# JGCRI/xanthos

Measured on AMD Instinct MI355X. Metric: cell-months/sec (pm_abcd_mrtm, 67,420 cells), higher is better.
Workload: dtype f64

## Files before the change

include/xanthos_hip.h:

```cpp
#ifndef XANTHOS_HIP_H
#define XANTHOS_HIP_H

#include <stddef.h>
#include <stdint.h>

#ifdef __cplusplus
extern "C" {
#endif

#define XH_OK 0
#define XH_ERR_ARG 1
#define XH_ERR_HIP 2
#define XH_ERR_LIMIT 3
#define XH_ERR_DEVICE 4

#define XH_MAX_LCS 32

typedef struct xh_ctx xh_ctx;
typedef struct xh_route_plan xh_route_plan;

int xh_abi_version(void);
int xh_device_count(int *n);
int xh_ctx_create(int device, xh_ctx **out);
void xh_ctx_destroy(xh_ctx *ctx);
// ... 83 lines not shown

int xh_gwam(xh_ctx *ctx, int64_t ncell, int32_t nmonths, int32_t spinup, int32_t precip_col_spinup,
            int32_t precip_col_sim, double indexing,
            const double *d_pet, const double *d_precip,
            const double *d_sm_max, const double *d_sm0,
            double *d_aet, double *d_q, double *d_sav,
            double *d_sm_end);

int xh_route_plan_create(xh_ctx *ctx, int64_t ncell, const int64_t *h_indptr, const int32_t *h_indices,
                         const int8_t *h_sign, xh_route_plan **out);
void xh_route_plan_destroy(xh_route_plan *plan);
int xh_route_plan_info(const xh_route_plan *plan, int64_t info[16]);

int xh_route_plan_prepare(xh_ctx *ctx, xh_route_plan *plan, const double *h_flow_dist, const double *h_velocity, double dt);

int xh_route_plan_stats(xh_route_plan *plan, int64_t max_words, uint64_t *h_words, int64_t *n_words);

int xh_mrtm_downstream(int64_t ncell, int32_t nrow, int32_t ncol, const int64_t *h_id, const int32_t *h_ilon,
                       const int32_t *h_ilat, const double *h_flowdir, int64_t *h_dsid);
int xh_mrtm_upstream(int64_t ncell, int32_t nrow, int32_t ncol, const int64_t *h_id, const int32_t *h_ilon,
                     const int32_t *h_ilat, const int64_t *h_dsid, int64_t *h_upid);
int xh_mrtm_um_csr(int64_t ncell, const int64_t *h_upid, int64_t *h_indptr, int32_t *h_indices, int8_t *h_sign);

#define XH_ROUTE_DEFAULT 0
#define XH_ROUTE_FORCE_FALLBACK 1
#define XH_ROUTE_ATOMIC 2
#define XH_ROUTE_NO_DATAFLOW 4
#define XH_ROUTE_NO_SKEW 8
#define XH_ROUTE_TEST_FAULT 16
#define XH_ROUTE_VALIDATE 32
#define XH_ROUTE_REASSOC 128
#define XH_ROUTE_EXACT 256
int xh_route_plan_rsum_info(const xh_route_plan *plan, int64_t info[8]);
int xh_route_series(xh_ctx *ctx, xh_route_plan *plan, int32_t nmonths, int32_t spinup_months,
                    const int32_t *h_ndays, double dt,
                    const double *d_flow_dist, const double *d_velocity, const double *d_area,
                    const double *d_runoff, const double *d_S0,
                    double *d_chstorage, double *d_avgchflow, double *d_S_end, double *d_F_end, int32_t flags);

typedef struct xh_fused_args {
    int64_t ncell;
    int32_t nmonths, start_year;
    const xh_pm_tables *pm;
    int32_t n_lc_years;
    const int32_t *h_lc_years;
    int32_t water_idx, snow_idx;
    const double *d_tas, *d_tmin, *d_rhs, *d_wind, *d_rsds, *d_rlds, *d_tairprev, *d_lct, *d_elev;
    int32_t abcd_spinup, n_groups;
    const int32_t *h_basin_index, *h_par_index;
    int64_t npar_rows;
    const double *d_pars, *d_precip, *d_abcd_tmin;
    xh_route_plan *plan;
    int32_t routing_spinup;
    const int32_t *h_ndays;
    double dt;
    const double *d_flow_dist, *d_velocity, *d_area, *d_S0;
    int32_t route_flags;
    double *d_pet, *d_aet, *d_q, *d_sav, *d_chstorage, *d_avgchflow;
    int32_t block_months;
    int32_t mode;
} xh_fused_args;
int xh_run_fused(xh_ctx *ctx, const xh_fused_args *args);

int xh_calib_objective(xh_ctx *ctx, int64_t ncell_b, int32_t nmonths, int32_t spinup, int32_t nmembers,
                       int32_t npar, const double *h_pars, const double *d_pet_t, const double *d_precip_t,
                       const double *d_tmin_t, const double *d_area, const double *h_obs, double *h_ed,
// ... 163 lines not shown
```

xanthos_amd/_hip.py:

```python
import contextlib
import ctypes
import os
import threading
from ctypes import POINTER, Structure, byref, c_char_p, c_double, c_int, c_int8, c_int32, c_int64, c_size_t, \
    c_uint64, c_void_p

import numpy as np

_HERE = os.path.dirname(os.path.abspath(__file__))
LIB_PATH = os.environ.get('XH_LIBRARY') or os.path.join(_HERE, 'libxanthos_hip.so')

XH_ROUTE_DEFAULT, XH_ROUTE_FORCE_FALLBACK, XH_ROUTE_ATOMIC, XH_ROUTE_NO_DATAFLOW, XH_ROUTE_NO_SKEW = 0, 1, 2, 4, 8
XH_ROUTE_TEST_FAULT, XH_ROUTE_VALIDATE = 16, 32
XH_ROUTE_REASSOC, XH_ROUTE_EXACT = 128, 256
XH_ROUTE_NO_PLAIN = 0x4000
XH_DAYLIGHT_REFERENCE, XH_DAYLIGHT_MONTHLY = 0, 1
XH_ERR_ARG, XH_ERR_HIP, XH_ERR_LIMIT, XH_ERR_DEVICE = 1, 2, 3, 4
ENS_STAT_BITS = {'mean': 1, 'std': 2, 'min': 4, 'max': 8}


class HipUnavailable(RuntimeError):
    """The HIP library or device is not usable; nothing falls back to the CPU."""


# ... 70 lines not shown
    'xh_memcpy_d2d': (c_int, [_P, _P, _P, c_size_t]),
    'xh_host_alloc': (c_int, [_P, c_size_t, POINTER(c_void_p)]),
    'xh_host_free': (c_int, [_P, _P]),
    'xh_memcpy_h2d_async': (c_int, [_P, _P, _P, c_size_t]),
    'xh_memcpy_d2h_async': (c_int, [_P, _P, _P, c_size_t]),
    'xh_upload_file': (c_int, [_P, _P, c_char_p, ctypes.c_uint64, c_size_t, c_int]),
    'xh_download_file': (c_int, [_P, _P, c_char_p, ctypes.c_uint64, c_size_t, c_int]),
    'xh_download_files': (c_int, [_P, c_int, POINTER(c_void_p), POINTER(c_char_p), POINTER(ctypes.c_uint64), POINTER(c_size_t)]),
    'xh_csv_format': (c_int, [_P, _P, c_int64, c_int64, c_int64, _P, c_size_t, _P]),
    'xh_csv_write': (c_int, [_P, _P, c_int64, c_int64, c_int64, c_char_p, ctypes.c_uint64, c_size_t, POINTER(ctypes.c_uint64)]),
    'xh_csv_write_many': (c_int, [_P, c_int, POINTER(c_void_p), POINTER(c_int64), POINTER(c_int64), POINTER(c_int64),
                                  POINTER(c_char_p), POINTER(ctypes.c_uint64), c_size_t, POINTER(ctypes.c_uint64)]),
    'xh_pack_f32_be': (c_int, [_P, _P, c_int64, _P]),
    'xh_memset': (c_int, [_P, _P, c_int, c_size_t]),
    'xh_sync': (c_int, [_P]),
    'xh_gather_rows': (c_int, [_P, _P, _P, c_int64, c_int64, _P]),
    'xh_scatter_rows': (c_int, [_P, _P, _P, c_int64, c_int64, _P]),
    'xh_transpose': (c_int, [_P, _P, c_int64, c_int64, _P]),
    'xh_timing_reset': (c_int, [_P]),
    'xh_timing_enable': (c_int, [_P, c_int]),
    'xh_timing_get': (c_int, [_P, c_char_p, POINTER(c_double), POINTER(c_int64)]),
    'xh_pm_pet': (c_int, [_P, POINTER(PmTables), c_int64, c_int32, c_int32, c_int32, _P, c_int32, c_int32,
                          _P, _P, _P, _P, _P, _P, _P, _P, _P, _P]),
    'xh_abcd': (c_int, [_P, c_int64, c_int32, c_int32, c_int32, _P, _P, c_int64, _P, _P, _P, _P, _P, _P, _P, _P, _P]),
    'xh_hargreaves_pet': (c_int, [_P, c_int64, c_int32, _P, _P, _P, _P, _P, _P, _P]),
    'xh_gwam': (c_int, [_P, c_int64, c_int32, c_int32, c_int32, c_int32, c_double, _P, _P, _P, _P, _P, _P, _P, _P]),
    'xh_hs_pet': (c_int, [_P, c_int64, c_int32, _P, _P, _P, _P, _P, _P]),
    'xh_thornthwaite_pet': (c_int, [_P, c_int64, c_int32, c_int32, c_int32, _P, _P, _P, _P]),
    'xh_route_plan_create': (c_int, [_P, c_int64, _P, _P, _P, POINTER(c_void_p)]),
    'xh_route_plan_destroy': (None, [_P]),
    'xh_route_plan_info': (c_int, [_P, POINTER(c_int64)]),
    'xh_route_plan_stats': (c_int, [_P, c_int64, _P, POINTER(c_int64)]),
    'xh_route_plan_rsum_info': (c_int, [_P, POINTER(c_int64)]),
    'xh_route_plan_prepare': (c_int, [_P, _P, _P, _P, c_double]),
    'xh_mrtm_downstream': (c_int, [c_int64, c_int32, c_int32, _P, _P, _P, _P, _P]),
    'xh_mrtm_upstream': (c_int, [c_int64, c_int32, c_int32, _P, _P, _P, _P, _P]),
    'xh_mrtm_um_csr': (c_int, [c_int64, _P, _P, _P, _P]),
    'xh_route_series': (c_int, [_P, _P, c_int32, c_int32, _P, c_double, _P, _P, _P, _P, _P, _P, _P, _P, _P, c_int32]),
    'xh_run_fused': (c_int, [_P, POINTER(FusedArgs)]),
    'xh_calib_objective': (c_int, [_P, c_int64, c_int32, c_int32, c_int32, c_int32, _P, _P, _P, _P, _P, _P, _P, _P]),
    'xh_calib_objective_multi': (c_int, [_P, c_int32, _P, c_int32, c_int32, c_int32, c_int32, _P, _P, _P, _P, _P, _P, _P, _P]),
    'xh_calib_de_create': (c_int, [_P, c_int32, _P, _P, c_int32, c_int32, c_int32, c_int32, _P, _P, _P, _P, _P, _P, _P,
                                   c_uint64, POINTER(c_void_p)]),
    'xh_calib_flow_objective_multi': (c_int, [_P, c_int32, _P, c_int32, c_int32, c_int32, c_int32, _P, _P, _P, _P,
                                              POINTER(CalibFlowDesc), _P, _P, _P]),
    'xh_calib_de_create_flow': (c_int, [_P, c_int32, _P, _P, c_int32, c_int32, c_int32, c_int32, _P, _P, _P,
                                        POINTER(CalibFlowDesc), _P, _P, _P, c_uint64, POINTER(c_void_p)]),
    'xh_calib_gauge_objective_multi': (c_int, [_P, c_int32, _P, c_int32, c_int32, c_int32, c_int32, _P, _P, _P, _P,
                                               POINTER(CalibGaugeDesc), _P, _P, _P, _P]),
    'xh_calib_de_create_gauge': (c_int, [_P, c_int32, _P, _P, c_int32, c_int32, c_int32, c_int32, _P, _P, _P,
                                         POINTER(CalibGaugeDesc), _P, _P, _P, c_uint64, POINTER(c_void_p)]),
    'xh_calib_flow_velocity_objective_multi': (c_int, [_P, c_int32, _P, c_int32, c_int32, c_int32, c_int32, _P, _P, _P, _P,
                                                       POINTER(CalibFlowDesc), POINTER(CalibVelocityDesc), _P, _P, _P]),
    'xh_calib_gauge_velocity_objective_multi': (c_int, [_P, c_int32, _P, c_int32, c_int32, c_int32, c_int32, _P, _P, _P, _P,
                                                        POINTER(CalibGaugeDesc), POINTER(CalibVelocityDesc), _P, _P, _P,
                                                        _P]),
    'xh_calib_de_create_flow_velocity': (c_int, [_P, c_int32, _P, _P, c_int32, c_int32, c_int32, c_int32, _P, _P, _P,
                                                 POINTER(CalibFlowDesc), POINTER(CalibVelocityDesc), _P, _P, _P, c_uint64,
                                                 POINTER(c_void_p)]),
    'xh_calib_de_create_gauge_velocity': (c_int, [_P, c_int32, _P, _P, c_int32, c_int32, c_int32, c_int32, _P, _P, _P,
                                                  POINTER(CalibGaugeDesc), POINTER(CalibVelocityDesc), _P, _P, _P, c_uint64,
                                                  POINTER(c_void_p)]),
    'xh_calib_de_destroy': (None, [_P]),
    'xh_calib_de_init': (c_int, [_P]),
    'xh_calib_de_step': (c_int, [_P, c_int32, c_double, c_double, c_double, c_double, c_double, POINTER(c_int32)]),
    'xh_calib_de_result': (c_int, [_P, _P, _P, _P, _P, _P]),
# ... 586 lines not shown


class RoutePlan:

    def __init__(self, ctx, indptr, indices, sign):
        self.ctx = ctx
        ip = np.ascontiguousarray(indptr, dtype=np.int64)
        ix = np.ascontiguousarray(indices, dtype=np.int32)
        sg = np.ascontiguousarray(sign, dtype=np.int8)
        self.ncell = ip.size - 1
        h = c_void_p()
        ctx._check(lib().xh_route_plan_create(ctx.handle, self.ncell, _host_ptr(ip), _host_ptr(ix), _host_ptr(sg),
                                              byref(h)))
        self.handle = h.value

    def info(self):
        arr = (c_int64 * 16)()
        self.ctx._check(lib().xh_route_plan_info(self.handle, arr))
        keys = ('networks', 'largest_network', 'units', 'fallback_cells', 'largest_unit', 'slots', 'single_downstream',
                'flow_units', 'flow_edges', 'flow_depth', 'flow_cells', 'flow_max_imports', 'skew_max_lag',
                'last_tree_kernel', 'reroutes', 'validated')
        return dict(zip(keys, list(arr)))

    def prepare(self, flow_dist, velocity, dt):
        L = np.ascontiguousarray(flow_dist, dtype=np.float64)
        v = np.ascontiguousarray(velocity, dtype=np.float64)
        if L.size != self.ncell or v.size != self.ncell:
            raise ValueError('flow_dist / velocity must have one value per cell')
        self.ctx._check(lib().xh_route_plan_prepare(self.ctx.handle, self.handle, _host_ptr(L), _host_ptr(v), float(dt)))

    def rsum_info(self):
        arr = (c_int64 * 8)()
        self.ctx._check(lib().xh_route_plan_rsum_info(self.handle, arr))
        return dict(zip(('units', 'folded', 'fold_disabled', 'prepared_folded', 'pair_cells', 'prepared_pair_cells', 'guard_trips',
                         'pair_units'), list(arr)))

    def stats(self):
        n = c_int64(0)
        self.ctx._check(lib().xh_route_plan_stats(self.handle, 0, None, byref(n)))
        if n.value == 0:
            return None
        out = np.empty(n.value, dtype=np.uint64)
        self.ctx._check(lib().xh_route_plan_stats(self.handle, n.value, _host_ptr(out), byref(n)))
        return out.reshape(-1, 6)

    def close(self):
        if self.handle is not None and self.ctx.handle is not None:
            lib().xh_route_plan_destroy(self.handle)
        self.handle = None

    def __del__(self):
        try:
            self.close()
        except Exception:
            pass


def comm_unique_id():
    buf = ctypes.create_string_buffer(128)
    _check_host(lib().xh_comm_unique_id(buf, 128))
    return buf.raw


class Comm:

    def __init__(self, ctx, nranks, rank, unique_id):
        self.ctx, self.nranks, self.rank = ctx, int(nranks), int(rank)
        h = c_void_p()
# ... 200 lines not shown
```

xanthos_amd/csrc/xh_flow_rsum.cpp:

```cpp
#include <algorithm>
#include <cstdio>
#include <numeric>
#include <string>
#include <thread>

#include "xh_flow_plan.h"

using xh_flow::Tree;
using xh_flow::tree_analyse;

namespace {

constexpr int LANES = 64;
constexpr int G_MAX = 16;
constexpr int W_MAX = 9;
constexpr int SK_P = 4;
constexpr unsigned SK_ZERO = 2u * LANES * 16u;
constexpr int H_MAX = 88;

struct RPart {
    std::vector<int> queue, piece, roots, psize, pimp, pdepth;
    std::vector<int> e_prod, e_cons, e_kind;
    std::vector<int> unit_of_piece, unit_cells, unit_imp, unit_out, unit_depth;
    std::vector<char> unit_cheap, unit_special, special, mayfire;
// ... 560 lines not shown
            hs[out.unit_p[u] & 3]++;
            hl[std::min(out.unit_lmax[u] / 16, 13)]++;
            hi[P.unit_imp[u] == 0 ? 0 : P.unit_imp[u] <= 2 ? 1 : P.unit_imp[u] <= 4 ? 2 : P.unit_imp[u] <= 8 ? 3 : 4]++;
            indep += (P.unit_imp[u] == 0 && unit_exp[u] == 0) ? 1 : 0;
        }
        fprintf(stderr, "flow plan (reassociated): %d units (%d without streams, %d kept cheap), %d pieces, %d streams, depth %d, %lld of %lld lanes used\n",
                nunit, indep, P.n_cheap, (int)roots.size(), nedge, P.maxdepth + 1, (long long)out.n_cells, (long long)ts);
        {
            int nfu = 0, nfi = 0;
            for (int u = 0; u < nunit; ++u) {
                nfu += (out.unit_p[u] & 4) ? 1 : 0;
                nfi += ((out.unit_p[u] & 4) && (P.unit_imp[u] > 0 || unit_exp[u] > 0)) ? 1 : 0;
            }
            fprintf(stderr, "  folded leaves: %d, in %d units (of them with streams: %d)\n", out.n_folded, nfu, nfi);
        }
        {
            int nsu = 0;
            for (int u = 0; u < nunit; ++u) nsu += (out.unit_p[u] & 16) ? 1 : 0;
            int nx = 0;
            for (int c = 0; c < n; ++c) nx += (P.n_special >= 0 && P.mayfire[c]) ? 1 : 0;
            int quiet = 0;
            for (int u = 0; u < nunit && P.n_special >= 0; ++u) {
                bool any = (out.unit_p[u] & 16) != 0;
                for (int k = 0; k < LANES && !any; ++k) any = (out.lane_flags[(int64_t)u * LANES + k] & 1) != 0;
                quiet += any ? 0 : 1;
            }
            for (int u = 0; u < nunit && P.n_special >= 0; ++u)
                if (out.unit_p[u] & 16)
                    fprintf(stderr, "  pair unit %d: %d cells, %d imports, %d outlets, depth %d, lmax %d\n", u, P.unit_cells[u], P.unit_imp[u], unit_exp[u],
                            P.unit_depth[u], out.unit_lmax[u]);
            fprintf(stderr, "  single-sum plan: %s, %d cells may fire, %d of them in pair form in %d units; %d single units hold no cell that may fire\n",
                    P.n_special >= 0 ? "yes" : "no", nx, std::max(P.n_special, 0), nsu, quiet);
        }
        fprintf(stderr, "  units by reads (none, A, R, A+R): %d %d %d %d\n  units by lmax/16 (0..13+):", hs[0], hs[1], hs[2], hs[3]);
        for (int k = 0; k < 14; ++k) fprintf(stderr, " %d", hl[k]);
        fprintf(stderr, "\n  units by imports (0, <=2, <=4, <=8, more): %d %d %d %d %d\n  longest stream jump: %d levels\n", hi[0], hi[1],
                hi[2], hi[3], hi[4], out.skew_span);
    }
    return 0;
}

std::string flow_tables_check_rsum(int n, const int64_t *indptr, const int32_t *indices, const int8_t *sign,
                                   const std::vector<char> &handled, const FlowTables &t) {
    if (!t.rsum) return "not a reassociated plan";
    if (t.n_units == 0) {
        for (int c = 0; c < n; ++c)
            if (handled[c]) return "handled cell without units";
        return "";
    }
    const int64_t ts = (int64_t)t.n_units * LANES;
    if ((int64_t)t.cell_of_slot.size() != ts || (int64_t)t.lag.size() != ts || (int64_t)t.eprev.size() != ts ||
        (int64_t)t.ent2.size() != 2 * SK_P * ts || (int)t.unit_p.size() != t.n_units || (int64_t)t.ghost_edge.size() != ts ||
        (int64_t)t.ghost_lag.size() != ts || (int64_t)t.export_edge.size() != ts || (int)t.unit_lmax.size() != t.n_units ||
        (int)t.unit_order.size() != t.n_units || (int)t.edge_cons_unit.size() != t.n_edges ||
        (int)t.edge_prod_cell.size() != t.n_edges || (int)t.edge_cons_cell.size() != t.n_edges || (int)t.ds.size() != n ||
        (int)t.unit_depth.size() != t.n_units)
        return "table sizes";
    std::vector<int> slot_of(n, -1);
    for (int64_t s = 0; s < ts; ++s) {
        const int c = t.cell_of_slot[s];
        if (c < 0) continue;
        if (c >= n || !handled[c]) return "slot holds a cell that is not handled";
        if (slot_of[c] >= 0) return "cell " + std::to_string(c) + " sits in two slots";
        slot_of[c] = (int)s;
    }
    std::vector<int> carrier(n, -1);
// ... 148 lines not shown
```

xanthos_amd/csrc/xh_mrtm.hip:

```cpp
#include <algorithm>
#include <chrono>
#include <climits>
#include <cmath>
#include <atomic>
#include <numeric>
#include <thread>

#include "xh_common.h"
#include <sys/stat.h>
#include <unistd.h>

#include "xh_mrtm_flow.h"
#include "xh_mrtm_plan.h"

namespace {

constexpr int W_MAX = 9;
constexpr int W_BASE = 3;
constexpr int UNIT_MAX_CELLS = 3072;
constexpr int BIN_CELLS = 256;
constexpr int N_CLASS = XH_ROUTE_N_CLASS;

struct UnitClass {
    int nt, kc;
// ... 747 lines not shown
            prepared.first_checked = false;
        }
        plan->fold_tried = true;
        plan->prep_key = key;
        plan->fold_disabled = false;
        const bool fold = fold_on && nfold > 0;
        if (!fold && !single_on) return XH_OK;
        const int rcu = rsum_partition(ctx, plan, fold ? foldable.data() : nullptr, single_on ? capable.data() : nullptr,
                                       &prepared.fp);
        if (rcu || !prepared.fp) return rcu;
        prepared.suffix = prepared.fp->n_special >= 0 ? "_rs" : "_rf";
        plan->fold_dt = dt;
        return XH_OK;
    }
    return XH_OK;
}

void xh_route_backoff(xh_route_plan *plan) {
    plan->fault_streak = std::min(plan->fault_streak + 1, 6);
    plan->skip_calls = 4 << plan->fault_streak;
}

extern "C" int xh_route_plan_rsum_info(const xh_route_plan *plan, int64_t info[8]) {
    if (!plan || !info) return XH_ERR_ARG;
    const FlowPlan *fp = last_reassoc(plan), *prep = plan->form[XH_FORM_PREPARED].fp;
    info[0] = fp ? fp->n_units : 0;
    info[1] = fp ? fp->n_folded : 0;
    info[2] = plan->fold_disabled ? 1 : 0;
    info[3] = prep ? prep->n_folded : 0;
    info[4] = fp ? fp->n_special : -1;
    info[5] = prep ? prep->n_special : -1;
    info[6] = plan->guard_trips;
    info[7] = fp ? fp->n_pair_units : 0;
    return XH_OK;
}

RouteChoice route_choose(const xh_route_plan *plan, int flags, double dt, bool fed) {
    RouteChoice c;
    c.whole_graph = (flags & XH_ROUTE_FORCE_FALLBACK) != 0;
    c.atomic = (flags & XH_ROUTE_ATOMIC) != 0;
    c.dataflow = !c.whole_graph && plan->form[XH_FORM_EXACT].fp && (flags & XH_ROUTE_NO_DATAFLOW) == 0;
    c.skew = (flags & XH_ROUTE_NO_SKEW) == 0;
    c.checkable = c.dataflow && !c.atomic && (flags & XH_ROUTE_TEST_FAULT) == 0;
    if (c.dataflow && c.skew && !c.atomic && reassoc_wanted(flags) && !plan->rsum_failed) {
        c.form = XH_FORM_PAIRS;
        if (plan->form[XH_FORM_PREPARED].fp && !plan->fold_disabled && dt == plan->fold_dt && (flags & XH_ROUTE_NO_PLAIN) == 0)
            c.form = XH_FORM_PREPARED;
    }
    c.refuse_fed = fed && (!c.dataflow || !c.skew || c.atomic || plan->n_rest_units > 0 || plan->fb_rest.n > 0);
    return c;
}

int route_series_impl(xh_ctx *ctx, xh_route_plan *plan, int32_t nmonths, int32_t spinup_months,
                             const int32_t *h_ndays, double dt, const double *d_flow_dist, const double *d_velocity,
                             const double *d_area, const double *d_runoff, const double *d_S0, double *d_chstorage,
                             double *d_avgchflow, double *d_S_end, double *d_F_end, int32_t flags, xh_route_outcome *out,
                             const FlowFeed *feed) {
    if (!ctx || !plan) return XH_ERR_ARG;
    XH_REQUIRE(ctx, plan->ctx == ctx, "xh_route_series: plan belongs to another context");
    XH_REQUIRE(ctx, h_ndays && d_flow_dist && d_velocity && d_area && d_runoff, "xh_route_series: NULL argument");
    XH_REQUIRE(ctx, nmonths > 0 && spinup_months >= 0 && spinup_months <= nmonths,
               "xh_route_series: need 0 <= spinup_months (%d) <= nmonths (%d)", spinup_months, nmonths);
    XH_REQUIRE(ctx, dt > 0.0, "xh_route_series: dt must be positive");
    if (plan->ncell == 0) return XH_OK;

    const int nit = spinup_months + nmonths;
// ... 205 lines not shown
```

xanthos_amd/csrc/xh_mrtm_flow.h:

```cpp
#pragma once
#include <functional>
#include <string>
#include <vector>

#include "xh_common.h"
#include "xh_flow_plan.h"

struct FlowBuf {
    void *p = nullptr;
};

struct FlowPlan {
    int n_units = 0, n_edges = 0, depth = 0, n_cells = 0, max_imports = 0, max_exports = 0;
    bool rsum = false;
    int max_cell = -1;
    FlowBuf d_cell_of_slot, d_ent, d_export_edge, d_ghost_edge, d_edge_cons_unit, d_unit_terms;
    bool skew_ok = false;
    int skew_lmax = 0;
    int skew_span = 1;
    FlowBuf d_lag, d_ghost_lag, d_ent2, d_eprev, d_unit_p, d_unit_lmax, d_unit_glmax, d_unit_order;
    void *d_x = nullptr;
    size_t x_bytes = 0;
    unsigned long long *d_stats = nullptr;
    void *d_skew_args = nullptr;
    std::vector<char> h_rec, h_fin;
    uint64_t rec_key = 0;
    FlowBuf d_fold_cell;
    int n_folded = 0;
    int n_special = -1;
    int n_pair_units = 0;
    FlowBuf d_lane_flags;
};

struct FlowSched {
    int nmonths, nit, ntmax, ntmin, total;
    const int *d_m, *d_nt;
    const int *d_g;
    const double *d_secs;
    const unsigned char *d_wr;
    double dt;
    bool test_fault;
    bool nt_even;
    const int *h_m, *h_nt, *h_g;
    const double *h_secs;
    const unsigned char *h_wr;
};

struct FlowFeed {
    const double *q_staged = nullptr;
    int64_t ncell = 0;
    const unsigned *months_ready = nullptr;
    unsigned ready_at_launch = 0;
    unsigned *place_epoch = nullptr;
    unsigned epoch = 0;
};

struct FlowIO {
    const double *flow_dist, *velocity, *area, *runoff, *S0;
    double *chs, *avg, *S_end, *F_end;
    const FlowFeed *feed = nullptr;
};

int flow_plan_build(xh_ctx *ctx, int n, const int64_t *indptr, const int32_t *indices, const int8_t *sign, uint64_t topo_hash,
                    const std::vector<int> &comp, int ncomp, std::vector<char> &handled, FlowPlan **out);
// ... 15 lines not shown
```

xanthos_amd/csrc/xh_mrtm_flow.hip:

```cpp

#include <algorithm>
#include <cmath>
#include <cstdlib>
#include <numeric>

#include "xh_flow_plan.h"
#include "xh_mrtm_flow.h"

namespace {

constexpr int W_MAX = 9;
constexpr int LANES = 64;
constexpr int NPAIR = 2 * LANES + 1;
constexpr int RING = 4;
constexpr int PF = 8;
constexpr unsigned FAULT_DATA_WAIT = 1, FAULT_RING_WAIT = 2;
constexpr unsigned FAULT_TEST = 99;
constexpr unsigned long long SPIN_LIMIT_TICKS = 500000000ull;

struct FlowArgs {
    const int *cell_of_slot;
    const unsigned *ent;
    const int *export_edge;
    const int *ghost_edge;
// ... 316 lines not shown
    if (t.n_units == 0) return XH_OK;
    FlowPlan *fp = new FlowPlan();
    fp->skew_ok = t.skew_ok;
    fp->skew_lmax = t.skew_lmax;
    fp->skew_span = t.skew_span;
    fp->n_units = t.n_units;
    fp->n_edges = t.n_edges;
    fp->depth = t.depth;
    fp->n_cells = t.n_cells;
    fp->max_imports = t.max_imports;
    fp->max_exports = t.max_exports;
    fp->rsum = t.rsum;
    for (int c : t.cell_of_slot) fp->max_cell = std::max(fp->max_cell, c);
    for (int c : t.fold_of_slot) fp->max_cell = std::max(fp->max_cell, c);
    int rc = put(ctx, fp->d_cell_of_slot, t.cell_of_slot);
    rc |= put(ctx, fp->d_ent, t.ent);
    rc |= put(ctx, fp->d_export_edge, t.export_edge);
    rc |= put(ctx, fp->d_ghost_edge, t.ghost_edge);
    rc |= put(ctx, fp->d_edge_cons_unit, t.edge_cons_unit);
    rc |= put(ctx, fp->d_unit_terms, t.unit_terms);
    rc |= put(ctx, fp->d_lag, t.lag);
    rc |= put(ctx, fp->d_ghost_lag, t.ghost_lag);
    rc |= put(ctx, fp->d_ent2, t.ent2);
    rc |= put(ctx, fp->d_eprev, t.eprev);
    rc |= put(ctx, fp->d_unit_p, t.unit_p);
    rc |= put(ctx, fp->d_unit_order, t.unit_order);
    rc |= put(ctx, fp->d_unit_lmax, t.unit_lmax);
    rc |= put(ctx, fp->d_unit_glmax, t.unit_glmax);
    rc |= put(ctx, fp->d_lane_flags, t.lane_flags);
    if (!t.fold_of_slot.empty()) rc |= put(ctx, fp->d_fold_cell, t.fold_of_slot);
    fp->n_folded = t.n_folded;
    fp->n_special = t.n_special;
    fp->n_pair_units = t.n_pair_units;
    if (rc) {
        flow_plan_destroy(fp);
        return XH_ERR_HIP;
    }
    *out = fp;
    return XH_OK;
}

int flow_stats_fetch(xh_ctx *ctx, FlowPlan *fp, std::vector<unsigned long long> &out) {
    out.clear();
    if (!fp || !fp->d_stats) return XH_OK;
    out.resize((size_t)fp->n_units * 6);
    XH_HIP(ctx, hipStreamSynchronize(ctx->stream));
    XH_HIP(ctx, hipMemcpy(out.data(), fp->d_stats, out.size() * 8, hipMemcpyDeviceToHost));
    return XH_OK;
}

int flow_launch(xh_ctx *ctx, FlowPlan *fp, const FlowSched &s, const FlowIO &io, hipStream_t st) {
    if (!fp || fp->n_units == 0) return XH_OK;
    const size_t x_streams = (size_t)std::max(fp->n_edges, 1) * RING * (size_t)s.ntmax * sizeof(double2);
    const size_t x_cnt = ((size_t)(fp->n_edges + fp->n_units) * sizeof(unsigned) + 255) & ~size_t(255);
    fp->rec_key = 0;
    if (x_streams + x_cnt > fp->x_bytes) {
        if (fp->d_x) {
            XH_HIP(ctx, hipStreamSynchronize(st));
            XH_HIP(ctx, hipFree(fp->d_x));
            fp->d_x = nullptr;
        }
        XH_HIP(ctx, hipMalloc(&fp->d_x, x_streams + x_cnt));
        fp->x_bytes = x_streams + x_cnt;
    }
    unsigned *cnt = reinterpret_cast<unsigned *>(static_cast<char *>(fp->d_x) + x_streams);
    XH_HIP(ctx, hipMemsetAsync(cnt, 0, x_cnt, st));
// ... 61 lines not shown
```

xanthos_amd/csrc/xh_mrtm_rsum.hip:

```cpp
#include <algorithm>
#include "xh_mrtm_wave_unit.h"

namespace {

__global__ void __launch_bounds__(LANES) __attribute__((amdgpu_waves_per_eu(2, 2))) k_mrtm_rsum(const WaveArgs *ap_) {
    WaveArgsK *ap = (WaveArgsK *)ap_;
    __shared__ __attribute__((aligned(16))) v2d lds[RING * NSLOT];
    __shared__ uint2 xtab[LANES];
    __shared__ unsigned qstage_sh[4 * LANES];
    __shared__ double fend_sh[2 * LANES];
    __shared__ int unit_sh, prio_sh;
    const int unit = wave_claim(ap, &unit_sh, &prio_sh);
    const int prio = prio_sh;
    if (unit < 0) return;
    if (A(months_ready)) {
        if (prio == 3) __builtin_amdgcn_s_setprio(3);
        else if (prio == 1) __builtin_amdgcn_s_setprio(1);
        else __builtin_amdgcn_s_setprio(2);
    } else if (prio == 3) {
        __builtin_amdgcn_s_setprio(3);
    }
    const int p = A(unit_p)[unit];
    const bool has_ghost = A(ghost_edge)[(int64_t)unit * LANES + threadIdx.x] >= 0;
    const bool g = __any(has_ghost), g2 = __any(has_ghost && threadIdx.x >= 8);
    const int nxo = __popcll(__ballot(A(export_edge)[(int64_t)unit * LANES + threadIdx.x] >= 0));
    const bool x = nxo > 0;
    char *l = reinterpret_cast<char *>(lds);
    __attribute__((address_space(3))) unsigned *qst = (__attribute__((address_space(3))) unsigned *)qstage_sh;
    __attribute__((address_space(3))) double *fnd = (__attribute__((address_space(3))) double *)fend_sh;
    fend_sh[threadIdx.x] = 0.0;
    fend_sh[LANES + threadIdx.x] = 0.0;
    if ((p & ~31) != 0x400) {
        if (threadIdx.x == 0) __hip_atomic_store(A(fault), FAULT_PLACE_WAIT, __ATOMIC_RELAXED, __HIP_MEMORY_SCOPE_AGENT);
        return;
    }
    bool bad = false;
#define XH_BY_OUTLETS(...)                                                                 \
    do {                                                                                   \
        if (nxo > 8) wave_unit<__VA_ARGS__, -1>(ap, l, xtab, qst, fnd, unit);              \
        else if (x) wave_unit<__VA_ARGS__, 1>(ap, l, xtab, qst, fnd, unit);                \
        else wave_unit<__VA_ARGS__, 0>(ap, l, xtab, qst, fnd, unit);                       \
    } while (0)
    if (p & 16) {
        if (!(p & 8) || (p & 4)) bad = true;
        else if (g2) XH_BY_OUTLETS(1, 0, 2, true, true, false, 2);
        else if (g) XH_BY_OUTLETS(1, 0, 1, true, true, false, 2);
        else XH_BY_OUTLETS(1, 0, 0, true, true, false, 2);
#undef XH_BY_OUTLETS
    } else if (p & 8) {
        if (p & 4) {
            if (g || !A(fold_cell)) bad = true;
            else wave_unit<1, 0, 0, true, true, true, 1>(ap, l, xtab, qst, fnd, unit);
        } else if (g2) wave_unit<1, 0, 2, true, true, false, 1>(ap, l, xtab, qst, fnd, unit);
        else if (g) wave_unit<1, 0, 1, true, true, false, 1>(ap, l, xtab, qst, fnd, unit);
        else if ((p & 2) || x) wave_unit<1, 0, 0, true, true, false, 1>(ap, l, xtab, qst, fnd, unit);
        else if (p & 1) wave_unit<1, 0, 0, false, true, false, 1>(ap, l, xtab, qst, fnd, unit);
        else wave_unit<0, 0, 0, false, true, false, 1>(ap, l, xtab, qst, fnd, unit);
    } else if (p & 4) {
        if (g || !A(fold_cell)) bad = true;
        else wave_unit<1, 0, 0, true, true, true>(ap, l, xtab, qst, fnd, unit);
    } else if (g2) wave_unit<1, 0, 2, true, true>(ap, l, xtab, qst, fnd, unit);
    else if (g) wave_unit<1, 0, 1, true, true>(ap, l, xtab, qst, fnd, unit);
    else if ((p & 2) || x) wave_unit<1, 0, 0, true, true>(ap, l, xtab, qst, fnd, unit);
    else if (p & 1) wave_unit<1, 0, 0, false, true>(ap, l, xtab, qst, fnd, unit);
    else wave_unit<0, 0, 0, false, true>(ap, l, xtab, qst, fnd, unit);
    if (bad && threadIdx.x == 0)
        __hip_atomic_store(A(fault), FAULT_PLACE_WAIT, __ATOMIC_RELAXED, __HIP_MEMORY_SCOPE_AGENT);
}
#undef A

}

const void *wave_rsum_kernel() { return reinterpret_cast<const void *>(&k_mrtm_rsum); }
```

xanthos_amd/csrc/xh_mrtm_wave_unit.h:

```cpp
#pragma once
#include <algorithm>
#include <climits>
#include <cstdlib>
#include <type_traits>

#include "xh_mrtm_flow.h"

namespace {


constexpr int LANES = 64;
constexpr int SK_P = 4;
#ifndef XH_WAVE_MIDZONE
#define XH_WAVE_MIDZONE 1
#endif
#ifndef XH_WAVE_BMOV
#define XH_WAVE_BMOV 1
#endif
constexpr int NSLOT = 2 * LANES + 1;
constexpr int RING = 8;
constexpr int GROUP = 16;
constexpr int SK_R = 2;
#ifndef XH_WAVE_CH
#define XH_WAVE_CH 256
// ... 124 lines not shown
    typedef typename V::lds_c lds_cv;
    typedef typename V::lds_m lds_mv;
    constexpr unsigned VB = V::B;
    constexpr unsigned SLOTB = NSLOT * VB;
    lds_char *lds0 = (lds_char *)lds_generic;
    const int lane = threadIdx.x;
    const int64_t slot = (int64_t)unit * LANES + lane;

    const int gc = A(cell_of_slot)[slot];
    const bool valid = gc >= 0;
    const int gc_safe = valid ? gc : 0;
    const unsigned row_off = (unsigned)gc_safe * A(q_row_stride);
    const double tauinv = valid ? A(velocity)[gc] / A(flow_dist)[gc] : 0.0;
    const double acoef = 1.0 - tauinv * A(dt);
    const double area = valid ? A(area)[gc] : 0.0;
    const double S0v = (valid && A(S0)) ? A(S0)[gc] : 0.0;
    auto ent_off = [](unsigned o) { return V8 ? o >> 1 : o; };
    static_assert(!RSUM || (PRE <= 1 && POST == 0), "reassociated form: one inflow entry");
    static_assert(!FOLD || (RSUM && NG == 0), "folded leaves: reassociated form, units without imports");
    static_assert(SGL == 0 || RSUM, "single-sum plans: reassociated form");
    const int gcL = FOLD ? A(fold_cell)[slot] : -1;
    const bool validL = FOLD && valid && gcL >= 0;
    const unsigned row_offL = (unsigned)(validL ? gcL : 0) * A(q_row_stride);
    const double tauL = validL ? A(velocity)[gcL] / A(flow_dist)[gcL] : 0.0;
    const double acoefL = 1.0 - tauL * A(dt);
    const double areaL = validL ? A(area)[gcL] : 0.0;
    const double S0L = (validL && A(S0)) ? A(S0)[gcL] : 0.0;
    double SL = 0.0, favgL = 0.0, erlL = 0.0, erlL_n = 0.0, snapSL = 0.0, snapAL = 0.0, FL = 0.0;
    constexpr double FOLD_EPS = 1e-6;
    unsigned gfold = (validL && !(tauL * A(dt) <= 1.0 - 1.0 / 1048576.0 && tauL >= 0.0 && S0L >= 0.0)) ? 1u : 0u;
    constexpr double SGL_EPS = 1e-6;
    constexpr double SGL_XEPS = 1e-10;
    unsigned gsgl = 0;
    bool xlane = false;
    double fmin_seen = 0.0;
    if (SGL != 0) {
        const unsigned lf = A(lane_flags)[slot];
        xlane = valid && (lf & 2u) != 0;
        gsgl = (valid && (!(tauinv >= 0.0) || (!(tauinv * A(dt) <= 1.0 - 1.0 / 1048576.0) && !(lf & 1u)) || S0v < 0.0)) ? 1u : 0u;
    }
    constexpr int PRE_N = PRE > 0 ? PRE : 1, POST_N = POST > 0 ? POST : 1;
    lds_cchar *epre[PRE_N], *epost[POST_N];
#pragma unroll
    for (int w = 0; w < PRE; ++w) epre[w] = lds0 + ent_off(A(ent2)[(int64_t)w * A(total_slots) + slot]);
#pragma unroll
    for (int w = 0; w < POST; ++w) epost[w] = lds0 + ent_off(A(ent2)[(int64_t)(SK_P + w) * A(total_slots) + slot]);
    lds_cchar *eprv = lds0 + (CHAIN ? ent_off(A(eprev)[slot]) : 0u);
    lds_mv *own = (lds_mv *)lds0 + lane;
    const int xedge = A(export_edge)[slot];
    const int gedge = A(ghost_edge)[slot];
    const bool has_x = xedge >= 0, has_g = gedge >= 0;
    const unsigned long long xmask = __ballot(has_x), gmask = __ballot(has_g);
    const int nx_out = __popcll(xmask), ng = __popcll(gmask);
    static_assert(NXR >= -1 && NXR <= 1, "outlet rounds known at compile time: none or one");
    const bool any_x = NXR < 0 ? xmask != 0 : NXR > 0, any_g = HAS_G;
    const int lmax = A(unit_lmax)[unit], glmax = A(unit_glmax)[unit];
    const int lag_g = has_g ? A(ghost_lag)[slot] : 0;
    const unsigned *ready_p = A(ready) + (has_g ? gedge : 0);
    const unsigned *done_p = A(done) + (has_x ? A(edge_cons_unit)[xedge] : 0);
    const unsigned maskb = A(ring_mask_b);
    const unsigned oob = ~maskb;
    const __amdgpu_buffer_rsrc_t xr = __builtin_amdgcn_make_buffer_rsrc(A(xbuf), 0, (int)A(xbytes), 0x00020000);
    const int total = A(total), nit = A(nit);
    const bool odd_ok = A(odd_ok) != 0;

    if (has_x) xtab[__popcll(xmask & ((1ull << lane) - 1ull))] = make_uint2((unsigned)lane, (unsigned)xedge);
    const int sub = lane & 7, grp = lane >> 3;
    const bool x2 = NXR < 0 && nx_out > 8;
    unsigned gfull[SK_R], xbyte[SK_R];
    lds_mv *gdst[SK_R];
    lds_cv *xsrc[SK_R];
// ... 91 lines not shown
    constexpr int OB = 4;
    double ob_s[OB], ob_a[OB];
    double ob_sL[FOLD ? OB : 1], ob_aL[FOLD ? OB : 1];
#pragma unroll
    for (int j = 0; j < OB; ++j) ob_s[j] = ob_a[j] = 0.0;
#pragma unroll
    for (int j = 0; j < (FOLD ? OB : 1); ++j) ob_sL[j] = ob_aL[j] = 0.0;
    bool alive = true;
    unsigned mready = A(ready_at_launch);
    auto wait_months = [&](unsigned need) {
        const unsigned *p = A(months_ready);
        if (!p) return true;
        const unsigned long long t0 = __builtin_amdgcn_s_memrealtime();
        for (;;) {
            unsigned v = 0;
            if (lane == 0) v = __hip_atomic_fetch_add(const_cast<unsigned *>(p), 0u, __ATOMIC_RELAXED, __HIP_MEMORY_SCOPE_AGENT);
            v = (unsigned)__builtin_amdgcn_readfirstlane((int)v);
            if (v >= need) {
                mready = v;
                return true;
            }
            if (ld_relaxed(A(fault)) != 0) return false;
            if (__builtin_amdgcn_s_memrealtime() - t0 > SPIN_LIMIT_TICKS) {
                __hip_atomic_store(A(fault), FAULT_DATA_WAIT, __ATOMIC_RELAXED, __HIP_MEMORY_SCOPE_AGENT);
                return false;
            }
            __builtin_amdgcn_s_sleep(16);
        }
    };
    unsigned long long cyc_wait_data = 0, cyc_wait_ring = 0, zone_groups = 0;
    const unsigned long long cyc_begin = __builtin_amdgcn_s_memtime();
    const unsigned long long rt_begin = __builtin_amdgcn_s_memrealtime();

    unsigned seen_ready = 0, seen_done = 0, pend_ready = 0, pend_done = 0;
    auto load_async = [&](const unsigned *q) {
        unsigned v;
        asm volatile("global_load_dword %0, %1, off sc1" : "=v"(v) : "v"(q) : "memory");
        return v;
    };
    auto check = [&](int n) {
        const unsigned long long w0 = __builtin_amdgcn_s_memtime();
        asm volatile("s_waitcnt vmcnt(8)" : "+v"(pend_ready), "+v"(pend_done) : : "memory");
        asm volatile("s_waitcnt vmcnt(0)" ::: "memory");
        if (SGL == 2) gsgl |= (xlane && fmin_seen < -SGL_XEPS) ? 4u : 0u;
        if ((FOLD && __any(gfold != 0)) || (SGL != 0 && __any(gsgl != 0))) {
            __hip_atomic_store(A(fault), FAULT_GUARD, __ATOMIC_RELAXED, __HIP_MEMORY_SCOPE_AGENT);
            alive = false;
        }
        const bool fenced = A(fenced) == 1;
        if (any_x) {
            const int pub = min(max(n - RING - lmax, 0), total);
            if (fenced) __builtin_amdgcn_fence(__ATOMIC_RELEASE, "agent");
            if (has_x) __hip_atomic_store(A(ready) + xedge, (unsigned)pub, __ATOMIC_RELAXED, __HIP_MEMORY_SCOPE_AGENT);
            const int need = n + CH - lmax - A(rs);
            seen_done = max(seen_done, pend_done);
            if (need > 0 && alive)
                alive = wave_wait_ge(has_x, done_p, (unsigned)min(need, total), seen_done, A(fault), FAULT_RING_WAIT);
        }
        const unsigned long long w1 = __builtin_amdgcn_s_memtime();
        if (any_g && alive) {
            if (lane == 0)
                __hip_atomic_store(A(done) + unit, (unsigned)min(max(n - glmax, 0), total), __ATOMIC_RELAXED,
                                   __HIP_MEMORY_SCOPE_AGENT);
            const int need = min(total, n + CH + GROUP - lag_g);
            seen_ready = max(seen_ready, pend_ready);
            alive = wave_wait_ge(has_g && need > 0, ready_p, (unsigned)max(need, 0), seen_ready, A(fault), FAULT_DATA_WAIT);
            if (fenced) __builtin_amdgcn_fence(__ATOMIC_ACQUIRE, "agent");
            asm volatile("" ::: "memory");
        }
        if (any_x) pend_done = load_async(done_p);
        if (any_g) pend_ready = load_async(ready_p);
        cyc_wait_ring += w1 - w0;
        cyc_wait_data += __builtin_amdgcn_s_memtime() - w1;
    };

    auto finalize = [&](int it) {
        const FinRec f = fc;
        fc = ld_fin(it + 1 <= nit ? it + 1 : nit + 1);
        if (it + 1 < nit) {
            const double qn = runoff_take();
            erl_n = ((valid ? qn : 0.0) * area) * 1000.0 / f.secs_next1;
            if (RSUM) erl_n *= dt;
            if (SGL != 0) gsgl |= (erl_n < -SGL_EPS) ? 2u : 0u;
            if (FOLD) {
                const unsigned lo = qstage[2 * LANES + lane], hi = qstage[3 * LANES + lane];
                const double qnL = __hiloint2double((int)hi, (int)lo);
                erlL_n = (((validL ? qnL : 0.0) * areaL) * 1000.0 / f.secs_next1) * dt;
            }
        }
        if (it >= 1) {
            const int m = f.m_prev_w & (FIN_WRITE - 1);
            const bool write_prev = (f.m_prev_w & FIN_WRITE) != 0;
#pragma unroll
            for (int j = 0; j < OB - 1; ++j) {
                ob_s[j] = ob_s[j + 1];
                ob_a[j] = ob_a[j + 1];
            }
            ob_s[OB - 1] = snapS;
            ob_a[OB - 1] = snapA / (double)f.nt_prev;
            if (FOLD) {
#pragma unroll
                for (int j = 0; j < OB - 1; ++j) {
                    ob_sL[j] = ob_sL[j + 1];
                    ob_aL[j] = ob_aL[j + 1];
// ... 291 lines not shown
        }
    }
    if (alive) {
        if (any_x) {
            const unsigned xpos = ((unsigned)(N - RING - lmax) * 16u) & maskb;
            store_pair(*xsrc[0], xbyte[0], xpos);
            if (x2) store_pair(*xsrc[1], xbyte[1], xpos);
            asm volatile("s_waitcnt vmcnt(0)" ::: "memory");
            if (A(fenced) == 1) __builtin_amdgcn_fence(__ATOMIC_RELEASE, "agent");
            if (has_x) __hip_atomic_store(A(ready) + xedge, (unsigned)total, __ATOMIC_RELAXED, __HIP_MEMORY_SCOPE_AGENT);
        }
        if (any_g && lane == 0)
            __hip_atomic_store(A(done) + unit, (unsigned)total, __ATOMIC_RELAXED, __HIP_MEMORY_SCOPE_AGENT);
        if (valid) {
            if (A(S_end)) A(S_end)[gc] = snapS;
            if (A(F_end)) A(F_end)[gc] = fend[lane];
        }
        if (validL) {
            if (A(S_end)) A(S_end)[gcL] = snapSL;
            if (A(F_end)) A(F_end)[gcL] = fend[LANES + lane];
        }
    }
    const bool guard_set = __any((gfold | gsgl) != 0);
    if (A(stats) && lane == 0) {
        unsigned long long *st = A(stats) + (int64_t)unit * 6;
        const unsigned long long cyc = __builtin_amdgcn_s_memtime() - cyc_begin;
        st[0] = cyc - cyc_wait_data - cyc_wait_ring;
        st[1] = cyc;
        st[2] = __builtin_amdgcn_s_memrealtime() - rt_begin;
        const unsigned hw = __builtin_amdgcn_s_getreg((4) | (0 << 6) | (31 << 11));
        const unsigned xcc = __builtin_amdgcn_s_getreg((20) | (0 << 6) | (3 << 11));
        st[3] = (unsigned long long)((PRE + POST + (CHAIN ? 1 : 0) + 1) & 15) | (any_g ? 16u : 0u) | (any_x ? 32u : 0u) |
                (V8 ? 64u : 0u) | (guard_set ? 128u : 0u) | ((unsigned long long)hw << 8) | ((unsigned long long)(xcc & 15u) << 40) |
                (zone_groups << 44);
        st[4] = cyc_wait_data;
        st[5] = cyc_wait_ring;
#ifdef XH_WAVE_PROFILE
        st[0] = prof_plain;
        st[4] = prof_zone;
        st[5] = prof_fin;
#endif
    }
}


__device__ __forceinline__ int wave_claim(WaveArgsK *ap, int *unit_sh_p, int *prio_sh_p) {
    int &unit_sh = *unit_sh_p, &prio_sh = *prio_sh_p;
    if (threadIdx.x == 0) {
        prio_sh = 0;
        unsigned *pl = A(place);
        const unsigned hw = __builtin_amdgcn_s_getreg((4) | (0 << 6) | (31 << 11));
        const unsigned xcc = __builtin_amdgcn_s_getreg((20) | (0 << 6) | (3 << 11)) & 15u;
        const unsigned key = ((((xcc * 8u + ((hw >> 13) & 7u)) * 2u + ((hw >> 12) & 1u)) * 16u + ((hw >> 8) & 15u)) * 4u) +
                             ((hw >> 4) & 3u);
        unsigned *pl_cu = pl + 16 + PLACE_KEYS + (key >> 2);
        const int n_units = A(n_units);
        const unsigned n_wg = gridDim.x;
        unsigned *fault = A(fault);
        auto wait_for = [&](unsigned *word, unsigned target) {
            const unsigned long long t0 = __builtin_amdgcn_s_memrealtime();
            while (__hip_atomic_load(word, __ATOMIC_ACQUIRE, __HIP_MEMORY_SCOPE_AGENT) < target) {
                if (ld_relaxed(fault) != 0 || __builtin_amdgcn_s_memrealtime() - t0 > SPIN_LIMIT_TICKS) {
                    __hip_atomic_store(fault, FAULT_PLACE_WAIT, __ATOMIC_RELAXED, __HIP_MEMORY_SCOPE_AGENT);
                    return false;
                }
                __builtin_amdgcn_s_sleep(8);
            }
// ... 81 lines not shown
```

Baseline: 3.153 billion.

## Stage ring counters through LDS and specialize single-sum units by outlet count

The asynchronous loads of the ready/done ring counters now use global_load_lds_dword into an LDS staging area (reusing xtab), so they no longer tie up VGPRs across the wait and check reads them back from LDS. Single-sum units are now dispatched through the outlet-count templates (0, <=8, >8 outlets), the same way paired units already were, so units with few or no outlets get a cheaper specialized path. Diagnostics for outlet shape counts and extra stats bits are added. This risks LDS aliasing with other uses of xtab, and the inline asm that saves and restores m0 is fragile.

Result: no change. 3.186 billion, median of 3 (+1.1%).

```diff
diff --git a/include/xanthos_hip.h b/include/xanthos_hip.h
--- a/include/xanthos_hip.h
+++ b/include/xanthos_hip.h
@@ -139,6 +139,7 @@
 #define XH_ROUTE_REASSOC 128
 #define XH_ROUTE_EXACT 256
 int xh_route_plan_rsum_info(const xh_route_plan *plan, int64_t info[8]);
+int xh_route_plan_rsum_shapes(const xh_route_plan *plan, int64_t info[3]);
 int xh_route_series(xh_ctx *ctx, xh_route_plan *plan, int32_t nmonths, int32_t spinup_months,
                     const int32_t *h_ndays, double dt,
                     const double *d_flow_dist, const double *d_velocity, const double *d_area,
diff --git a/xanthos_amd/_hip.py b/xanthos_amd/_hip.py
--- a/xanthos_amd/_hip.py
+++ b/xanthos_amd/_hip.py
@@ -126,6 +126,7 @@
     'xh_route_plan_info': (c_int, [_P, POINTER(c_int64)]),
     'xh_route_plan_stats': (c_int, [_P, c_int64, _P, POINTER(c_int64)]),
     'xh_route_plan_rsum_info': (c_int, [_P, POINTER(c_int64)]),
+    'xh_route_plan_rsum_shapes': (c_int, [_P, POINTER(c_int64)]),
     'xh_route_plan_prepare': (c_int, [_P, _P, _P, _P, c_double]),
     'xh_mrtm_downstream': (c_int, [c_int64, c_int32, c_int32, _P, _P, _P, _P, _P]),
     'xh_mrtm_upstream': (c_int, [c_int64, c_int32, c_int32, _P, _P, _P, _P, _P]),
@@ -778,8 +779,12 @@
     def rsum_info(self):
         arr = (c_int64 * 8)()
         self.ctx._check(lib().xh_route_plan_rsum_info(self.handle, arr))
-        return dict(zip(('units', 'folded', 'fold_disabled', 'prepared_folded', 'pair_cells', 'prepared_pair_cells', 'guard_trips',
-                         'pair_units'), list(arr)))
+        out = dict(zip(('units', 'folded', 'fold_disabled', 'prepared_folded', 'pair_cells', 'prepared_pair_cells', 'guard_trips',
+                        'pair_units'), list(arr)))
+        shp = (c_int64 * 3)()
+        self.ctx._check(lib().xh_route_plan_rsum_shapes(self.handle, shp))
+        out.update(zip(('single_no_outlet', 'single_outlets_le8', 'single_outlets_gt8'), list(shp)))
+        return out
 
     def stats(self):
         n = c_int64(0)
diff --git a/xanthos_amd/csrc/xh_flow_rsum.cpp b/xanthos_amd/csrc/xh_flow_rsum.cpp
--- a/xanthos_amd/csrc/xh_flow_rsum.cpp
+++ b/xanthos_amd/csrc/xh_flow_rsum.cpp
@@ -616,6 +616,12 @@
             fprintf(stderr, "  single-sum plan: %s, %d cells may fire, %d of them in pair form in %d units; %d single units hold no cell that may fire\n",
                     P.n_special >= 0 ? "yes" : "no", nx, std::max(P.n_special, 0), nsu, quiet);
         }
+        {
+            int xo[3] = {0, 0, 0};
+            for (int u = 0; u < nunit && P.n_special >= 0; ++u)
+                if (!(out.unit_p[u] & 16)) xo[unit_exp[u] == 0 ? 0 : unit_exp[u] <= 8 ? 1 : 2]++;
+            fprintf(stderr, "  single units by outlets (none, <= 8, more): %d %d %d\n", xo[0], xo[1], xo[2]);
+        }
         fprintf(stderr, "  units by reads (none, A, R, A+R): %d %d %d %d\n  units by lmax/16 (0..13+):", hs[0], hs[1], hs[2], hs[3]);
         for (int k = 0; k < 14; ++k) fprintf(stderr, " %d", hl[k]);
         fprintf(stderr, "\n  units by imports (0, <=2, <=4, <=8, more): %d %d %d %d %d\n  longest stream jump: %d levels\n", hi[0], hi[1],
diff --git a/xanthos_amd/csrc/xh_mrtm.hip b/xanthos_amd/csrc/xh_mrtm.hip
--- a/xanthos_amd/csrc/xh_mrtm.hip
+++ b/xanthos_amd/csrc/xh_mrtm.hip
@@ -803,6 +803,13 @@
     info[5] = prep ? prep->n_special : -1;
     info[6] = plan->guard_trips;
     info[7] = fp ? fp->n_pair_units : 0;
+    return XH_OK;
+}
+
+extern "C" int xh_route_plan_rsum_shapes(const xh_route_plan *plan, int64_t info[3]) {
+    if (!plan || !info) return XH_ERR_ARG;
+    const FlowPlan *fp = last_reassoc(plan);
+    for (int k = 0; k < 3; ++k) info[k] = fp ? fp->n_single_out[k] : 0;
     return XH_OK;
 }
 
diff --git a/xanthos_amd/csrc/xh_mrtm_flow.h b/xanthos_amd/csrc/xh_mrtm_flow.h
--- a/xanthos_amd/csrc/xh_mrtm_flow.h
+++ b/xanthos_amd/csrc/xh_mrtm_flow.h
@@ -30,6 +30,7 @@
     int n_special = -1;
     int n_pair_units = 0;
     FlowBuf d_lane_flags;
+    int n_single_out[3] = {0, 0, 0};
 };
 
 struct FlowSched {
diff --git a/xanthos_amd/csrc/xh_mrtm_flow.hip b/xanthos_amd/csrc/xh_mrtm_flow.hip
--- a/xanthos_amd/csrc/xh_mrtm_flow.hip
+++ b/xanthos_amd/csrc/xh_mrtm_flow.hip
@@ -372,6 +372,13 @@
     fp->n_folded = t.n_folded;
     fp->n_special = t.n_special;
     fp->n_pair_units = t.n_pair_units;
+    if (t.rsum && t.n_special >= 0)
+        for (int u = 0; u < t.n_units; ++u) {
+            if ((t.unit_p[u] & 24) != 8) continue;
+            int nx = 0;
+            for (int k = 0; k < LANES; ++k) nx += t.export_edge[(int64_t)u * LANES + k] >= 0 ? 1 : 0;
+            fp->n_single_out[nx == 0 ? 0 : (nx <= 8 ? 1 : 2)] += 1;
+        }
     if (rc) {
         flow_plan_destroy(fp);
         return XH_ERR_HIP;
diff --git a/xanthos_amd/csrc/xh_mrtm_rsum.hip b/xanthos_amd/csrc/xh_mrtm_rsum.hip
--- a/xanthos_amd/csrc/xh_mrtm_rsum.hip
+++ b/xanthos_amd/csrc/xh_mrtm_rsum.hip
@@ -35,27 +35,37 @@
         return;
     }
     bool bad = false;
+#ifndef XH_RSUM_SINGLE_NXR
+#define XH_RSUM_SINGLE_NXR 1
+#endif
+    constexpr int NX0 = XH_RSUM_SINGLE_NXR ? 0 : -1;
 #define XH_BY_OUTLETS(...)                                                                 \
     do {                                                                                   \
         if (nxo > 8) wave_unit<__VA_ARGS__, -1>(ap, l, xtab, qst, fnd, unit);              \
         else if (x) wave_unit<__VA_ARGS__, 1>(ap, l, xtab, qst, fnd, unit);                \
         else wave_unit<__VA_ARGS__, 0>(ap, l, xtab, qst, fnd, unit);                       \
     } while (0)
+#if XH_RSUM_SINGLE_NXR
+#define XH_SINGLE_BY_OUTLETS(...) XH_BY_OUTLETS(__VA_ARGS__)
+#else
+#define XH_SINGLE_BY_OUTLETS(...) wave_unit<__VA_ARGS__, -1>(ap, l, xtab, qst, fnd, unit)
+#endif
     if (p & 16) {
         if (!(p & 8) || (p & 4)) bad = true;
         else if (g2) XH_BY_OUTLETS(1, 0, 2, true, true, false, 2);
         else if (g) XH_BY_OUTLETS(1, 0, 1, true, true, false, 2);
         else XH_BY_OUTLETS(1, 0, 0, true, true, false, 2);
-#undef XH_BY_OUTLETS
     } else if (p & 8) {
         if (p & 4) {
             if (g || !A(fold_cell)) bad = true;
-            else wave_unit<1, 0, 0, true, true, true, 1>(ap, l, xtab, qst, fnd, unit);
-        } else if (g2) wave_unit<1, 0, 2, true, true, false, 1>(ap, l, xtab, qst, fnd, unit);
-        else if (g) wave_unit<1, 0, 1, true, true, false, 1>(ap, l, xtab, qst, fnd, unit);
-        else if ((p & 2) || x) wave_unit<1, 0, 0, true, true, false, 1>(ap, l, xtab, qst, fnd, unit);
-        else if (p & 1) wave_unit<1, 0, 0, false, true, false, 1>(ap, l, xtab, qst, fnd, unit);
-        else wave_unit<0, 0, 0, false, true, false, 1>(ap, l, xtab, qst, fnd, unit);
+            else XH_SINGLE_BY_OUTLETS(1, 0, 0, true, true, true, 1);
+        } else if (g2) XH_SINGLE_BY_OUTLETS(1, 0, 2, true, true, false, 1);
+        else if (g) XH_SINGLE_BY_OUTLETS(1, 0, 1, true, true, false, 1);
+        else if ((p & 2) || x) XH_SINGLE_BY_OUTLETS(1, 0, 0, true, true, false, 1);
+        else if (p & 1) wave_unit<1, 0, 0, false, true, false, 1, NX0>(ap, l, xtab, qst, fnd, unit);
+        else wave_unit<0, 0, 0, false, true, false, 1, NX0>(ap, l, xtab, qst, fnd, unit);
+#undef XH_SINGLE_BY_OUTLETS
+#undef XH_BY_OUTLETS
     } else if (p & 4) {
         if (g || !A(fold_cell)) bad = true;
         else wave_unit<1, 0, 0, true, true, true>(ap, l, xtab, qst, fnd, unit);
diff --git a/xanthos_amd/csrc/xh_mrtm_wave_unit.h b/xanthos_amd/csrc/xh_mrtm_wave_unit.h
--- a/xanthos_amd/csrc/xh_mrtm_wave_unit.h
+++ b/xanthos_amd/csrc/xh_mrtm_wave_unit.h
@@ -180,11 +180,12 @@
     constexpr double SGL_EPS = 1e-6;
     constexpr double SGL_XEPS = 1e-10;
     unsigned gsgl = 0;
-    bool xlane = false;
+    bool xlane = false, unit_mayfire = false;
     double fmin_seen = 0.0;
     if (SGL != 0) {
         const unsigned lf = A(lane_flags)[slot];
         xlane = valid && (lf & 2u) != 0;
+        unit_mayfire = __any(valid && (lf & 1u) != 0);
         gsgl = (valid && (!(tauinv >= 0.0) || (!(tauinv * A(dt) <= 1.0 - 1.0 / 1048576.0) && !(lf & 1u)) || S0v < 0.0)) ? 1u : 0u;
     }
     constexpr int PRE_N = PRE > 0 ? PRE : 1, POST_N = POST > 0 ? POST : 1;
@@ -342,16 +343,23 @@
     const unsigned long long cyc_begin = __builtin_amdgcn_s_memtime();
     const unsigned long long rt_begin = __builtin_amdgcn_s_memrealtime();
 
-    unsigned seen_ready = 0, seen_done = 0, pend_ready = 0, pend_done = 0;
-    auto load_async = [&](const unsigned *q) {
-        unsigned v;
-        asm volatile("global_load_dword %0, %1, off sc1" : "=v"(v) : "v"(q) : "memory");
-        return v;
+    unsigned seen_ready = 0, seen_done = 0;
+    __attribute__((address_space(3))) unsigned *cstage = (__attribute__((address_space(3))) unsigned *)xtab;
+    static_assert(sizeof(uint2) * LANES == 2 * LANES * sizeof(unsigned), "xtab holds the two counters of every lane");
+    cstage[lane] = 0u;
+    cstage[LANES + lane] = 0u;
+    const unsigned c_lds = (unsigned)(size_t)cstage;
+    auto load_async = [&](const unsigned *q, unsigned half) {
+        unsigned keep;
+        asm volatile("s_mov_b32 %0, m0\n\ts_mov_b32 m0, %2\n\tglobal_load_lds_dword %1, off sc1\n\ts_mov_b32 m0, %0"
+                     : "=&s"(keep)
+                     : "v"(q), "s"(c_lds + half * LANES * 4u)
+                     : "memory");
     };
     auto check = [&](int n) {
         const unsigned long long w0 = __builtin_amdgcn_s_memtime();
-        asm volatile("s_waitcnt vmcnt(8)" : "+v"(pend_ready), "+v"(pend_done) : : "memory");
         asm volatile("s_waitcnt vmcnt(0)" ::: "memory");
+        const unsigned pend_done = cstage[lane], pend_ready = cstage[LANES + lane];
         if (SGL == 2) gsgl |= (xlane && fmin_seen < -SGL_XEPS) ? 4u : 0u;
         if ((FOLD && __any(gfold != 0)) || (SGL != 0 && __any(gsgl != 0))) {
             __hip_atomic_store(A(fault), FAULT_GUARD, __ATOMIC_RELAXED, __HIP_MEMORY_SCOPE_AGENT);
@@ -378,8 +386,8 @@
             if (fenced) __builtin_amdgcn_fence(__ATOMIC_ACQUIRE, "agent");
             asm volatile("" ::: "memory");
         }
-        if (any_x) pend_done = load_async(done_p);
-        if (any_g) pend_ready = load_async(ready_p);
+        if (any_x) load_async(done_p, 0u);
+        if (any_g) load_async(ready_p, 1u);
         cyc_wait_ring += w1 - w0;
         cyc_wait_data += __builtin_amdgcn_s_memtime() - w1;
     };
@@ -737,7 +745,9 @@
         const unsigned xcc = __builtin_amdgcn_s_getreg((20) | (0 << 6) | (3 << 11));
         st[3] = (unsigned long long)((PRE + POST + (CHAIN ? 1 : 0) + 1) & 15) | (any_g ? 16u : 0u) | (any_x ? 32u : 0u) |
                 (V8 ? 64u : 0u) | (guard_set ? 128u : 0u) | ((unsigned long long)hw << 8) | ((unsigned long long)(xcc & 15u) << 40) |
-                (zone_groups << 44);
+                ((zone_groups & 0xffffull) << 44) |
+                (FOLD ? 1ull << 60 : 0ull) | (nx_out > 8 ? 1ull << 61 : 0ull) | (NG > 1 ? 1ull << 62 : 0ull) |
+                (unit_mayfire ? 1ull << 63 : 0ull);
         st[4] = cyc_wait_data;
         st[5] = cyc_wait_ring;
 #ifdef XH_WAVE_PROFILE
```
